# gabrielfnayres/new-vit

Hardware: AMD Instinct MI355X
Metric: volumes_per_sec_mst_dinov2_fwd (higher is better)
Workload: dtype bf16; 1 GPU; MST-DINOv2 (DinoV2ClassifierSlice, ViT-S/14) forward, 4 volumes/GPU of 64x512x512 bf16 zero-padded to 518x518 (N=1370 tokens/slice); global_batch_volumes=4, slices=64, parallelism=single GPU, weights=synthetic (mst.synth seed 2), random init of the reference architecture

## Files before the change

### new-vit_amd/csrc/k_attn16.hip

```cpp
#include <type_traits>

#include "mst_common.h"

namespace {

constexpr float LOG2E = 1.4426950408889634f;
constexpr int KV_TILE_BYTES = 64 * 128;
constexpr int K_ROW = 144, K_TILE_BYTES = 64 * K_ROW;

template <typename T>
__device__ __forceinline__ typename V8<T>::type tr_pair(const char* p_lo, const char* p_hi) {
    typedef typename V8<T>::type vec8;
    union { struct { s16x4 lo, hi; } s; vec8 v; } u;
    u.s.lo = __builtin_amdgcn_ds_read_tr16_b64_v4i16((__attribute__((address_space(3))) s16x4*)(p_lo));
    u.s.hi = __builtin_amdgcn_ds_read_tr16_b64_v4i16((__attribute__((address_space(3))) s16x4*)(p_hi));
    return u.v;
}

constexpr int ATTN_WG_WAVES = 4;
constexpr int WGW = ATTN_WG_WAVES, WGT = 64 * WGW, QB = 32 * WGW;
constexpr int ATTN_WAVES_PER_EU = 4;
template <typename T>
__global__ __launch_bounds__(WGT) __attribute__((amdgpu_waves_per_eu(ATTN_WAVES_PER_EU, ATTN_WAVES_PER_EU))) void attn16_kernel(const T* __restrict__ qkv, T* __restrict__ out,
                                                     int N, int heads, int log2q, int out_blocked) {
    typedef typename V8<T>::type vec8;
    __shared__ __attribute__((aligned(16))) char smem[4 * KV_TILE_BYTES];
    char* const Ks = smem;
    char* const Vs = smem + 2 * KV_TILE_BYTES;

    const int tid = threadIdx.x, lane = tid & 63;
    const int wave = __builtin_amdgcn_readfirstlane(tid >> 6);
    const int nqb = (N + QB - 1) / QB;
    const int tile = xcd_remap(blockIdx.x, gridDim.x);
    const int qb = tile % nqb, h = (tile / nqb) % heads, seq = tile / (nqb * heads);
    const int E = heads * 64, ld = 3 * E;
    const T* base = qkv + (int64_t)seq * N * ld;
    const int h2 = lane >> 5;

    const int q = qb * QB + wave * 32 + (lane & 31);
    const bool wave_active = (qb * QB + wave * 32) < N;
    vec8 bq[4];
    {
        const int qc = q < N ? q : N - 1;
        const T* qp = base + (int64_t)qc * ld + h * 64 + h2 * 8;
#pragma unroll
        for (int ds = 0; ds < 4; ++ds) bq[ds] = *reinterpret_cast<const vec8*>(qp + ds * 16);
    }

    static_assert(WGW == 4 || WGW == 8, "the LDS-DMA staging map deals 16 pieces per tile to 4 or 8 waves");
    constexpr int PPW = 16 / WGW;
    const int d_p0 = wave * PPW;
    const int d_row0 = (d_p0 & 7) * 8 + (lane >> 3);
    const int d_isv = d_p0 >> 3;
    const int d_chunk0 = d_isv ? ((lane & 7) ^ (((d_row0 >> 1) & 1) << 2)) : ((lane & 7) ^ ((d_row0 >> 1) & 7));
    const int d_col0 = (1 + d_isv) * (heads * 64) + h * 64 + d_chunk0 * 8;
    unsigned d_off[PPW];
#pragma unroll
    for (int u = 0; u < PPW; ++u) d_off[u] = (unsigned)(((d_row0 + 8 * u) * ld + ((u & 1) && !d_isv ? (d_col0 ^ 32) : d_col0)) * 2);
    auto dma = [&](int t, int buf) {
        char* dst = (d_isv ? Vs + buf * KV_TILE_BYTES : Ks + buf * KV_TILE_BYTES) + (d_p0 & 7) * 1024;
        if (t * 64 + 64 <= N) {
            const char* tb = reinterpret_cast<const char*>(base) + (int64_t)t * 64 * ld * 2;
#pragma unroll
            for (int u = 0; u < PPW; ++u) {
                const unsigned m0v = (unsigned)(size_t)(__attribute__((address_space(3))) char*)(dst + u * 1024);
#pragma clang diagnostic push
#pragma clang diagnostic ignored "-Winline-asm"
                asm volatile("s_mov_b32 m0, %2\n\ts_nop 0\n\tglobal_load_lds_dwordx4 %0, %1"
                             :
                             : "v"(d_off[u]), "s"(tb), "s"(m0v)
                             : "memory", "m0");
#pragma clang diagnostic pop
            }
        } else {
#pragma unroll
            for (int u = 0; u < PPW; ++u) {
                int key = t * 64 + d_row0 + 8 * u;
                key = key < N ? key : N - 1;
                const int col = (u & 1) && !d_isv ? (d_col0 ^ 32) : d_col0;
                __builtin_amdgcn_global_load_lds(GLB_PTR(base + (int64_t)key * ld + col), LDS_PTR(dst + u * 1024), 16, 0, 0);
            }
        }
    };
    const int krow = lane & 31;
    int k_off4[4];
#pragma unroll
    for (int ds = 0; ds < 4; ++ds) k_off4[ds] = krow * 128 + (((2 * ds + h2) ^ ((krow >> 1) & 7)) << 4);
    const int vi = lane & 15;
    const int vrow = 4 * h2 + (vi >> 2);
    const int vsw = ((vrow >> 1) & 1) << 2;
    const int vchunk = ((lane >> 4) & 1) * 2 + ((vi & 3) >> 1);
    const int v_lane_off = vrow * 128 + (vi & 1) * 8;

    f32x16 oT[2];
#pragma unroll
    for (int r = 0; r < 16; ++r) oT[0][r] = oT[1][r] = 0.f;
    if (!log2q) {
#pragma unroll
        for (int ds = 0; ds < 4; ++ds)
#pragma unroll
            for (int j = 0; j < 8; ++j) bq[ds][j] = (T)((float)bq[ds][j] * LOG2E);
    }
    float r_ref = 0.f, l_run = 0.f;
    constexpr float RT = 8.0f;

    const int nt = (N + 63) >> 6;
    dma(0, 0);
    asm volatile("s_waitcnt vmcnt(0)" ::: "memory");
    __syncthreads();

    constexpr float TH0 = std::is_same<T, f16_t>::value ? 8.0f : 60.0f;
    constexpr float GUARD = std::is_same<T, f16_t>::value ? 32768.0f : 1.2676506e30f;
    bool fast = false;

    auto tile_step = [&](auto mask_tag, auto fast_tag, int t, bool skip_dma) -> bool {
        constexpr bool MASK = decltype(mask_tag)::value;
        constexpr bool FAST = decltype(fast_tag)::value;
        const int buf = t & 1;
        if (t + 1 < nt && !skip_dma) dma(t + 1, buf ^ 1);
        if (wave_active) {
            const char* Kb = Ks + buf * KV_TILE_BYTES;
            const char* Vb = Vs + buf * KV_TILE_BYTES;
            f32x16 s[2];
            const f32x16 zero16 = {0.f, 0.f, 0.f, 0.f, 0.f, 0.f, 0.f, 0.f, 0.f, 0.f, 0.f, 0.f, 0.f, 0.f, 0.f, 0.f};
            const bool upper = !MASK || (t * 64 + 32 < N);
            auto scores = [&](bool with_ref) {
                vec8 kone, qneg;
                if (with_ref) {
#pragma unroll
                    for (int j = 0; j < 8; ++j) kone[j] = qneg[j] = (T)0.f;
                    if (h2 == 0) {
                        kone[0] = (T)1.f;
                        qneg[0] = (T)(-r_ref);
                    }
                }
#pragma unroll
                for (int kb = 0; kb < 2; ++kb) {
                    if (MASK && kb == 1 && !upper) {
#pragma unroll
                        for (int r = 0; r < 16; ++r) s[1][r] = -INFINITY;
                        continue;
                    }
                    s[kb] = with_ref ? mfma32(kone, qneg, zero16) : zero16;
#pragma unroll
                    for (int ds = 0; ds < 4; ++ds) {
                        const vec8 a = *reinterpret_cast<const vec8*>(Kb + k_off4[ds] + kb * 4096);
                        s[kb] = mfma32(a, bq[ds], s[kb]);
                    }
                }
                if constexpr (MASK) {
#pragma unroll
                    for (int kb = 0; kb < 2; ++kb)
#pragma unroll
                        for (int r = 0; r < 16; ++r) {
                            const int key = t * 64 + kb * 32 + (r & 3) + 8 * (r >> 2) + 4 * h2;
                            if (key >= N) s[kb][r] = -INFINITY;
                        }
                }
            };
            float lsum;
            vec8 pf[4];
            auto exps = [&]() {
                lsum = 0.f;
#pragma unroll
                for (int kb = 0; kb < 2; ++kb)
#pragma unroll
                    for (int r = 0; r < 16; ++r) {
                        const float p = __builtin_amdgcn_exp2f(s[kb][r]);
                        s[kb][r] = p;
                        lsum += p;
                    }
#pragma unroll
                for (int ks = 0; ks < 4; ++ks)
#pragma unroll
                    for (int j = 0; j < 8; ++j) pf[ks][j] = (T)s[ks >> 1][(ks & 1) * 8 + j];
            };
            auto classic = [&]() {
                float mx = s[0][0];
#pragma unroll
                for (int r = 1; r < 16; ++r) mx = fmaxf(mx, s[0][r]);
#pragma unroll
                for (int r = 0; r < 16; ++r) mx = fmaxf(mx, s[1][r]);
                {
                    const unsigned mu = __float_as_uint(mx);
                    const auto sw = __builtin_amdgcn_permlane32_swap(mu, mu, false, false);
                    mx = fmaxf(__uint_as_float(sw[0]), __uint_as_float(sw[1]));
                }
                if (t == 0 && __all(fabsf(mx) <= TH0)) {
                    fast = true;
                } else if (t == 0 || !__all(mx <= RT)) {
                    const bool mv = (t == 0) || (mx > RT);
                    const float r_new = mv ? (float)(T)(r_ref + mx) : r_ref;
                    const float delta = r_new - r_ref;
                    const float alpha = t == 0 ? 1.0f : __builtin_amdgcn_exp2f(-delta);
                    r_ref = r_new;
                    l_run *= alpha;
#pragma unroll
                    for (int r = 0; r < 16; ++r) {
                        oT[0][r] *= alpha;
                        oT[1][r] *= alpha;
                        s[0][r] -= delta;
                        s[1][r] -= delta;
                    }
                }
                exps();
            };
            if constexpr (FAST) {
                scores(false);
                exps();
                if (!__all(lsum < GUARD)) return false;
            } else {
                scores(true);
                classic();
            }
            l_run += lsum;
#pragma unroll
            for (int ks = 0; ks < 4; ++ks) {
                if (MASK && ks >= 2 && !upper) continue;
#pragma unroll
                for (int db = 0; db < 2; ++db) {
                    const char* p = Vb + ks * 16 * 128 + v_lane_off + (((db * 4 + vchunk) ^ vsw) * 16);
                    const vec8 vf = tr_pair<T>(p, p + 8 * 128);
                    oT[db] = mfma32(vf, pf[ks], oT[db]);
                }
            }
        }
        asm volatile("s_waitcnt vmcnt(0)" ::: "memory");
        __syncthreads();
        return true;
    };
    const int nt_full = (N & 63) ? nt - 1 : nt;
    const std::false_type FULL{}, CLASSIC{};
    const std::true_type RAGGED{}, FASTM{};
    if (nt_full > 0) tile_step(FULL, CLASSIC, 0, false);
    else tile_step(RAGGED, CLASSIC, 0, false);
    int t = 1;
    bool resume = false;
    if (fast) {
        for (; t < nt_full; ++t)
            if (!tile_step(FULL, FASTM, t, false)) { resume = true; break; }
    }
    for (; t < nt_full; ++t) {
        tile_step(FULL, CLASSIC, t, resume);
        resume = false;
    }
    if (t < nt) tile_step(RAGGED, CLASSIC, t, resume);

    if (wave_active) {
        const float l_tot = l_run + __shfl_xor(l_run, 32, 64);
        const float inv = 1.0f / l_tot;
        if (q < N) {
            const int64_t R = (int64_t)seq * N + q;
            T* op = out_blocked ? out + (R >> 5) * (32 * E) + (4 * h) * 512 + (R & 31) * 8 + 4 * h2
                                : out + R * E + h * 64 + 4 * h2;
            const int sdb = out_blocked ? 1024 : 32, sg2 = out_blocked ? 512 : 16, sg1 = out_blocked ? 256 : 8;
#pragma unroll
            for (int db = 0; db < 2; ++db)
#pragma unroll
                for (int g = 0; g < 4; ++g) {
                    typedef __attribute__((ext_vector_type(4))) T o4;
                    o4 pk;
#pragma unroll
                    for (int e = 0; e < 4; ++e) pk[e] = (T)(oT[db][g * 4 + e] * inv);
                    *reinterpret_cast<o4*>(op + db * sdb + (g >> 1) * sg2 + (g & 1) * sg1) = pk;
                }
        }
    }
}

template <typename T>
__global__ __launch_bounds__(256) void cls_probs_kernel(const T* __restrict__ qkv, float* __restrict__ probs,
                                                        int N, int heads, int hd, int log2q, T* __restrict__ attn_out = nullptr) {
    extern __shared__ float sm[];
    float* q0 = sm;
    float* sc = sm + hd;
    float* red = sc + N;
    const int h = blockIdx.x, seq = blockIdx.y, tid = threadIdx.x;
    const int E = heads * hd, ld = 3 * E;
    const T* base = qkv + (int64_t)seq * N * ld;
    for (int d = tid; d < hd; d += 256) q0[d] = to_f32(base[h * hd + d]);
    __syncthreads();
    float mx = -INFINITY;
    if (hd == 64) {
        const int sub = tid & 7;
        float qr[8];
#pragma unroll
        for (int i = 0; i < 8; ++i) qr[i] = q0[sub * 8 + i];
        for (int j0 = 0; j0 < N; j0 += 32) {
            const int j = j0 + (tid >> 3);
            const T* kp = base + (int64_t)(j < N ? j : N - 1) * ld + E + h * 64 + sub * 8;
            float a = 0.f;
#pragma unroll
            for (int i = 0; i < 8; ++i) a = fmaf(qr[i], to_f32(kp[i]), a);
            a += __shfl_xor(a, 1, 64);
            a += __shfl_xor(a, 2, 64);
            a += __shfl_xor(a, 4, 64);
            if (j < N) {
                if (sub == 0) sc[j] = a;
                mx = fmaxf(mx, a);
            }
        }
    } else {
        for (int j = tid; j < N; j += 256) {
            const T* kp = base + (int64_t)j * ld + E + h * hd;
            float a = 0.f;
            for (int d = 0; d < hd; ++d) a = fmaf(q0[d], to_f32(kp[d]), a);
            sc[j] = a;
            mx = fmaxf(mx, a);
        }
    }
    mx = wave_max(mx);
    if ((tid & 63) == 0) red[tid >> 6] = mx;
    __syncthreads();
    mx = fmaxf(fmaxf(red[0], red[1]), fmaxf(red[2], red[3]));
    float sum = 0.f;
    for (int j = tid; j < N; j += 256) {
        const float p = log2q ? exp2f(sc[j] - mx) : __expf(sc[j] - mx);
        sc[j] = p;
        sum += p;
    }
    sum = wave_sum(sum);
    if ((tid & 63) == 0) red[4 + (tid >> 6)] = sum;
    __syncthreads();
    const float inv = 1.0f / (red[4] + red[5] + red[6] + red[7]);
    if (probs) {
        float* po = probs + ((int64_t)seq * heads + h) * N;
        for (int j = tid; j < N; j += 256) po[j] = sc[j] * inv;
    }
    if (attn_out) {
        float* part = red + 8;
        const int d = tid & 63, pt = tid >> 6;
        const int per = (N + 3) >> 2;
        const int j1 = (pt + 1) * per < N ? (pt + 1) * per : N;
        float a = 0.f;
        for (int j = pt * per; j < j1; ++j) a = fmaf(sc[j], to_f32(base[(int64_t)j * ld + 2 * E + h * 64 + d]), a);
        part[pt * 64 + d] = a;
        __syncthreads();
        if (tid < 64) attn_out[(int64_t)seq * E + h * 64 + tid] = (T)(((part[tid] + part[64 + tid]) + (part[128 + tid] + part[192 + tid])) * inv);
    }
}

template <typename T>
__global__ __launch_bounds__(256) void probs_full_kernel(const T* __restrict__ qkv, float* __restrict__ probs,
                                                         int N, int heads, int hd, int log2q) {
    extern __shared__ float sm[];
    const int lane = threadIdx.x & 63, wave = threadIdx.x >> 6;
    float* qv = sm + wave * (hd + N);
    float* sc = qv + hd;
    const int h = blockIdx.y, seq = blockIdx.z;
    const int qi = blockIdx.x * 4 + wave;
    if (qi >= N) return;
    const int E = heads * hd, ld = 3 * E;
    const T* base = qkv + (int64_t)seq * N * ld;
    for (int d = lane; d < hd; d += 64) qv[d] = to_f32(base[(int64_t)qi * ld + h * hd + d]);
    __builtin_amdgcn_wave_barrier();
    float mx = -INFINITY;
    for (int j = lane; j < N; j += 64) {
        const T* kp = base + (int64_t)j * ld + E + h * hd;
        float a = 0.f;
        for (int d = 0; d < hd; ++d) a = fmaf(qv[d], to_f32(kp[d]), a);
        sc[j] = a;
        mx = fmaxf(mx, a);
    }
    mx = wave_max(mx);
    float sum = 0.f;
    for (int j = lane; j < N; j += 64) {
        const float p = log2q ? exp2f(sc[j] - mx) : __expf(sc[j] - mx);
        sc[j] = p;
        sum += p;
    }
    const float inv = 1.0f / wave_sum(sum);
    float* po = probs + (((int64_t)seq * heads + h) * N + qi) * N;
    for (int j = lane; j < N; j += 64) po[j] = sc[j] * inv;
}

template <typename T>
__global__ __launch_bounds__(256) void probs_full16_kernel(const T* __restrict__ qkv, float* __restrict__ probs, int N,
                                                           int heads, int log2q) {
    typedef typename V8<T>::type vec8;
    __shared__ __attribute__((aligned(16))) char smem[2 * K_TILE_BYTES + 128 * 8];
    char* const Ks = smem;
    float* const stat = reinterpret_cast<float*>(smem + 2 * K_TILE_BYTES);
    const int tid = threadIdx.x, lane = tid & 63;
    const int wave = __builtin_amdgcn_readfirstlane(tid >> 6);
    const int nqb = (N + 127) >> 7;
    const int tile = xcd_remap(blockIdx.x, gridDim.x);
    const int qb = tile % nqb, h = (tile / nqb) % heads, seq = tile / (nqb * heads);
    const int E = heads * 64, ld = 3 * E;
    const T* base = qkv + (int64_t)seq * N * ld;
    const int h2 = lane >> 5;
    const int q = qb * 128 + wave * 32 + (lane & 31);
    const float sc = log2q ? 1.0f : LOG2E;
    vec8 bq[4];
    {
        const int qc = q < N ? q : N - 1;
        const T* qp = base + (int64_t)qc * ld + h * 64 + h2 * 8;
#pragma unroll
        for (int ds = 0; ds < 4; ++ds) bq[ds] = *reinterpret_cast<const vec8*>(qp + ds * 16);
    }
    const int sr = tid >> 2, sc0 = (tid & 3) * 2;
    u32x4 rk0, rk1;
    auto gload = [&](int t) {
        int key = t * 64 + sr;
        key = key < N ? key : N - 1;
        const T* kp = base + (int64_t)key * ld + E + h * 64 + sc0 * 8;
        rk0 = *reinterpret_cast<const u32x4*>(kp);
        rk1 = *reinterpret_cast<const u32x4*>(kp + 8);
    };
    auto lstore = [&](int buf) {
        *reinterpret_cast<u32x4*>(Ks + buf * K_TILE_BYTES + sr * K_ROW + sc0 * 16) = rk0;
        *reinterpret_cast<u32x4*>(Ks + buf * K_TILE_BYTES + sr * K_ROW + sc0 * 16 + 16) = rk1;
    };
    const int k_lane_off = (lane & 31) * K_ROW + h2 * 16;
    const int nt = (N + 63) >> 6;
    const f32x16 zero16 = {0.f, 0.f, 0.f, 0.f, 0.f, 0.f, 0.f, 0.f, 0.f, 0.f, 0.f, 0.f, 0.f, 0.f, 0.f, 0.f};

    float m_run = -INFINITY, l_run = 0.f;
    gload(0);
    lstore(0);
    __syncthreads();
    for (int t = 0; t < nt; ++t) {
        const int buf = t & 1;
        if (t + 1 < nt) gload(t + 1);
        const char* Kb = Ks + buf * K_TILE_BYTES;
        f32x16 s[2];
#pragma unroll
        for (int kb = 0; kb < 2; ++kb) {
            s[kb] = zero16;
#pragma unroll
            for (int ds = 0; ds < 4; ++ds) {
                const vec8 a = *reinterpret_cast<const vec8*>(Kb + k_lane_off + kb * 32 * K_ROW + ds * 32);
                s[kb] = mfma32(a, bq[ds], s[kb]);
            }
        }
        float mx = -INFINITY;
#pragma unroll
        for (int kb = 0; kb < 2; ++kb)
#pragma unroll
            for (int r = 0; r < 16; ++r) {
                const int key = t * 64 + kb * 32 + (r & 3) + 8 * (r >> 2) + 4 * h2;
                s[kb][r] = key < N ? s[kb][r] * sc : -INFINITY;
                mx = fmaxf(mx, s[kb][r]);
            }
        mx = fmaxf(mx, __shfl_xor(mx, 32, 64));
        const float m_new = fmaxf(m_run, mx);
        float lsum = 0.f;
#pragma unroll
        for (int kb = 0; kb < 2; ++kb)
#pragma unroll
            for (int r = 0; r < 16; ++r) lsum += __builtin_amdgcn_exp2f(s[kb][r] - m_new);
        l_run = l_run * __builtin_amdgcn_exp2f(m_run - m_new) + lsum;
        m_run = m_new;
        if (t + 1 < nt) lstore(buf ^ 1);
        __syncthreads();
    }
    {
        const float l_tot = l_run + __shfl_xor(l_run, 32, 64);
        if (h2 == 0) {
            stat[(wave * 32 + (lane & 31)) * 2] = m_run;
            stat[(wave * 32 + (lane & 31)) * 2 + 1] = 1.0f / l_tot;
        }
    }
    __syncthreads();

    float mrow[16], irow[16];
#pragma unroll
    for (int r = 0; r < 16; ++r) {
        const int ql = wave * 32 + (r & 3) + 8 * (r >> 2) + 4 * h2;
        mrow[r] = stat[ql * 2];
        irow[r] = stat[ql * 2 + 1];
    }
    float* const pbase = probs + (((int64_t)seq * heads + h) * N) * N;
    gload(0);
    __syncthreads();
    lstore(0);
    __syncthreads();
    for (int t = 0; t < nt; ++t) {
        const int buf = t & 1;
        if (t + 1 < nt) gload(t + 1);
        const char* Kb = Ks + buf * K_TILE_BYTES;
#pragma unroll
        for (int kb = 0; kb < 2; ++kb) {
            f32x16 s = zero16;
#pragma unroll
            for (int ds = 0; ds < 4; ++ds) {
                const vec8 a = *reinterpret_cast<const vec8*>(Kb + k_lane_off + kb * 32 * K_ROW + ds * 32);
                s = mfma32(bq[ds], a, s);
            }
            const int key = t * 64 + kb * 32 + (lane & 31);
#pragma unroll
            for (int r = 0; r < 16; ++r) {
                const int qq = qb * 128 + wave * 32 + (r & 3) + 8 * (r >> 2) + 4 * h2;
                if (key < N && qq < N) pbase[(int64_t)qq * N + key] = __builtin_amdgcn_exp2f(s[r] * sc - mrow[r]) * irow[r];
            }
        }
        if (t + 1 < nt) lstore(buf ^ 1);
        __syncthreads();
    }
}

}

int launch_attn16(const void* qkv, int dt, int n_seq, int N, int heads, void* out, int log2q, hipStream_t s, int out_blocked) {
    MST_CHECK_ARG(n_seq > 0 && N > 0 && heads > 0, "attention: bad sizes n_seq=%d N=%d heads=%d", n_seq, N, heads);
    const int64_t nwg = (int64_t)((N + QB - 1) / QB) * heads * n_seq;
    MST_CHECK_ARG(nwg < (1ll << 31), "attention: grid too large");
    const dim3 grid((unsigned)nwg), block(WGT);
    if (dt == MST_BF16) attn16_kernel<bf16_t><<<grid, block, 0, s>>>((const bf16_t*)qkv, (bf16_t*)out, N, heads, log2q, out_blocked);
    else if (dt == MST_F16) attn16_kernel<f16_t><<<grid, block, 0, s>>>((const f16_t*)qkv, (f16_t*)out, N, heads, log2q, out_blocked);
    else { mst_set_error("attention16: bad dtype %d", dt); return MST_EINVAL; }
    return mst_check_launch("attention16");
}

int launch_cls_probs(const void* qkv, int dt, int n_seq, int N, int heads, int hd, float* probs, int log2q, hipStream_t s) {
    MST_CHECK_ARG(N > 0 && N <= 12000 && hd > 0 && hd <= 256, "cls_probs: N=%d hd=%d unsupported", N, hd);
    if (n_seq > 65535) {
        const size_t esz = dt == MST_F32 ? 4 : 2;
        for (int s0 = 0; s0 < n_seq; s0 += 65535) {
            const int c = (n_seq - s0 < 65535) ? n_seq - s0 : 65535;
            int rc = launch_cls_probs((const char*)qkv + (size_t)s0 * N * 3 * heads * hd * esz, dt, c, N, heads, hd,
                                      probs + (size_t)s0 * heads * N, log2q, s);
            if (rc) return rc;
        }
        return MST_OK;
    }
    const dim3 grid(heads, n_seq), block(256);
    const size_t sh = (size_t)(hd + N + 8 + 256) * sizeof(float);
    if (dt == MST_BF16) cls_probs_kernel<bf16_t><<<grid, block, sh, s>>>((const bf16_t*)qkv, probs, N, heads, hd, log2q);
    else if (dt == MST_F16) cls_probs_kernel<f16_t><<<grid, block, sh, s>>>((const f16_t*)qkv, probs, N, heads, hd, log2q);
    else if (dt == MST_F32) cls_probs_kernel<float><<<grid, block, sh, s>>>((const float*)qkv, probs, N, heads, hd, log2q);
    else { mst_set_error("cls_probs: bad dtype %d", dt); return MST_EINVAL; }
    return mst_check_launch("cls_probs");
}

int launch_cls_attn(const void* qkv, int dt, int n_seq, int N, int heads, float* probs, void* out, int log2q, hipStream_t s) {
    MST_CHECK_ARG(N > 0 && N <= 12000 && n_seq > 0 && n_seq <= 65535 && out, "cls_attn: N=%d n_seq=%d unsupported", N, n_seq);
    const dim3 grid(heads, n_seq), block(256);
    const size_t sh = (size_t)(64 + N + 8 + 256) * sizeof(float);
    if (dt == MST_BF16) cls_probs_kernel<bf16_t><<<grid, block, sh, s>>>((const bf16_t*)qkv, probs, N, heads, 64, log2q, (bf16_t*)out);
    else if (dt == MST_F16) cls_probs_kernel<f16_t><<<grid, block, sh, s>>>((const f16_t*)qkv, probs, N, heads, 64, log2q, (f16_t*)out);
    else if (dt == MST_F32) cls_probs_kernel<float><<<grid, block, sh, s>>>((const float*)qkv, probs, N, heads, 64, log2q, (float*)out);
    else { mst_set_error("cls_attn: bad dtype %d", dt); return MST_EINVAL; }
    return mst_check_launch("cls_attn");
}

int launch_probs_full(const void* qkv, int dt, int n_seq, int N, int heads, int hd, float* probs, int log2q, hipStream_t s) {
    if (hd == 64 && (dt == MST_BF16 || dt == MST_F16)) {
        MST_CHECK_ARG(N > 0 && n_seq > 0 && heads > 0, "probs_full: bad sizes");
        const int64_t nwg = (int64_t)((N + 127) / 128) * heads * n_seq;
        MST_CHECK_ARG(nwg < (1ll << 31), "probs_full: grid too large");
        if (dt == MST_BF16) probs_full16_kernel<bf16_t><<<dim3((unsigned)nwg), dim3(256), 0, s>>>((const bf16_t*)qkv, probs, N, heads, log2q);
        else probs_full16_kernel<f16_t><<<dim3((unsigned)nwg), dim3(256), 0, s>>>((const f16_t*)qkv, probs, N, heads, log2q);
        return mst_check_launch("probs_full16");
    }
    MST_CHECK_ARG(N > 0 && N <= 3800 && hd > 0 && hd <= 256, "probs_full: N=%d hd=%d unsupported", N, hd);
    if (n_seq > 65535) {
        const size_t esz = dt == MST_F32 ? 4 : 2;
        for (int s0 = 0; s0 < n_seq; s0 += 65535) {
            const int c = (n_seq - s0 < 65535) ? n_seq - s0 : 65535;
            int rc = launch_probs_full((const char*)qkv + (size_t)s0 * N * 3 * heads * hd * esz, dt, c, N, heads, hd,
                                       probs + (size_t)s0 * heads * N * N, log2q, s);
            if (rc) return rc;
        }
        return MST_OK;
    }
    const dim3 grid((N + 3) / 4, heads, n_seq), block(256);
    const size_t sh = (size_t)4 * (hd + N) * sizeof(float);
    if (dt == MST_BF16) probs_full_kernel<bf16_t><<<grid, block, sh, s>>>((const bf16_t*)qkv, probs, N, heads, hd, log2q);
    else if (dt == MST_F16) probs_full_kernel<f16_t><<<grid, block, sh, s>>>((const f16_t*)qkv, probs, N, heads, hd, log2q);
    else if (dt == MST_F32) probs_full_kernel<float><<<grid, block, sh, s>>>((const float*)qkv, probs, N, heads, hd, log2q);
    else { mst_set_error("probs_full: bad dtype %d", dt); return MST_EINVAL; }
    return mst_check_launch("probs_full");
}
```

Measured before the change: 163.5 volumes/s.

## Unroll attention KV loop by two with static buffers and MFMA row-sum

Unrolls the attention tile loop in pairs so the double-buffer index is a compile-time constant, hoists the V fragment offsets, and prefetches the first V fragments before the overflow guard check in the fast path. The softmax row sum moves from a scalar add chain plus a cross-lane shuffle to small MFMAs against a lane-selection vector. Inactive waves now run a separate loop that only issues DMA and barriers. The aim is to cut address arithmetic, VALU reduction work and the latency exposed at the guard. The cost is more control-flow complexity and a risk of barrier mismatch between active and inactive waves.

```diff
diff --git a/new-vit_amd/csrc/k_attn16.hip b/new-vit_amd/csrc/k_attn16.hip
--- a/new-vit_amd/csrc/k_attn16.hip
+++ b/new-vit_amd/csrc/k_attn16.hip
@@ -91,6 +91,10 @@
     const int vsw = ((vrow >> 1) & 1) << 2;
     const int vchunk = ((lane >> 4) & 1) * 2 + ((vi & 3) >> 1);
     const int v_lane_off = vrow * 128 + (vi & 1) * 8;
+    const int v_off2[2] = {v_lane_off + ((vchunk ^ vsw) << 4), v_lane_off + (((4 + vchunk) ^ vsw) << 4)};
+    vec8 sel;
+#pragma unroll
+    for (int j = 0; j < 8; ++j) sel[j] = (((lane >> 2) & 1) == ((lane >> 4) & 1)) ? (T)1.f : (T)0.f;
 
     f32x16 oT[2];
 #pragma unroll
@@ -113,12 +117,12 @@
     constexpr float GUARD = std::is_same<T, f16_t>::value ? 32768.0f : 1.2676506e30f;
     bool fast = false;
 
-    auto tile_step = [&](auto mask_tag, auto fast_tag, int t, bool skip_dma) -> bool {
+    auto tile_step = [&](auto mask_tag, auto fast_tag, auto buf_tag, int t, bool skip_dma) -> bool {
         constexpr bool MASK = decltype(mask_tag)::value;
         constexpr bool FAST = decltype(fast_tag)::value;
-        const int buf = t & 1;
+        const int buf = decltype(buf_tag)::value < 0 ? (t & 1) : decltype(buf_tag)::value;
         if (t + 1 < nt && !skip_dma) dma(t + 1, buf ^ 1);
-        if (wave_active) {
+        {
             const char* Kb = Ks + buf * KV_TILE_BYTES;
             const char* Vb = Vs + buf * KV_TILE_BYTES;
             f32x16 s[2];
@@ -158,22 +162,23 @@
                         }
                 }
             };
-            float lsum;
             vec8 pf[4];
+            f32x4 lsum;
             auto exps = [&]() {
-                lsum = 0.f;
 #pragma unroll
                 for (int kb = 0; kb < 2; ++kb)
 #pragma unroll
-                    for (int r = 0; r < 16; ++r) {
-                        const float p = __builtin_amdgcn_exp2f(s[kb][r]);
-                        s[kb][r] = p;
-                        lsum += p;
-                    }
+                    for (int r = 0; r < 16; ++r) s[kb][r] = __builtin_amdgcn_exp2f(s[kb][r]);
 #pragma unroll
                 for (int ks = 0; ks < 4; ++ks)
 #pragma unroll
                     for (int j = 0; j < 8; ++j) pf[ks][j] = (T)s[ks >> 1][(ks & 1) * 8 + j];
+                lsum = f32x4{0.f, 0.f, 0.f, 0.f};
+#pragma unroll
+                for (int ks = 0; ks < 4; ++ks) {
+                    if (MASK && ks >= 2 && !upper) continue;
+                    lsum = mfma16(sel, pf[ks], lsum);
+                }
             };
             auto classic = [&]() {
                 float mx = s[0][0];
@@ -205,22 +210,30 @@
                 }
                 exps();
             };
+            auto vfrag = [&](int ks, int db) {
+                const char* p = Vb + ks * 16 * 128 + v_off2[db];
+                return tr_pair<T>(p, p + 8 * 128);
+            };
             if constexpr (FAST) {
                 scores(false);
                 exps();
-                if (!__all(lsum < GUARD)) return false;
             } else {
                 scores(true);
                 classic();
             }
-            l_run += lsum;
+            vec8 vf0[2];
+            if constexpr (FAST) {
+                vf0[0] = vfrag(0, 0);
+                vf0[1] = vfrag(0, 1);
+                if (!__all(lsum[0] < GUARD)) return false;
+            }
+            l_run += lsum[0];
 #pragma unroll
             for (int ks = 0; ks < 4; ++ks) {
                 if (MASK && ks >= 2 && !upper) continue;
 #pragma unroll
                 for (int db = 0; db < 2; ++db) {
-                    const char* p = Vb + ks * 16 * 128 + v_lane_off + (((db * 4 + vchunk) ^ vsw) * 16);
-                    const vec8 vf = tr_pair<T>(p, p + 8 * 128);
+                    const vec8 vf = FAST && ks == 0 ? vf0[db] : vfrag(ks, db);
                     oT[db] = mfma32(vf, pf[ks], oT[db]);
                 }
             }
@@ -230,25 +243,53 @@
         return true;
     };
     const int nt_full = (N & 63) ? nt - 1 : nt;
+    if (!wave_active) {
+        for (int t = 0; t < nt; ++t) {
+            if (t + 1 < nt) dma(t + 1, (t + 1) & 1);
+            asm volatile("s_waitcnt vmcnt(0)" ::: "memory");
+            __syncthreads();
+        }
+        return;
+    }
     const std::false_type FULL{}, CLASSIC{};
     const std::true_type RAGGED{}, FASTM{};
-    if (nt_full > 0) tile_step(FULL, CLASSIC, 0, false);
-    else tile_step(RAGGED, CLASSIC, 0, false);
+    const std::integral_constant<int, 0> B0{};
+    const std::integral_constant<int, 1> B1{};
+    const std::integral_constant<int, -1> BDYN{};
+    if (nt_full > 0) tile_step(FULL, CLASSIC, B0, 0, false);
+    else tile_step(RAGGED, CLASSIC, B0, 0, false);
     int t = 1;
     bool resume = false;
     if (fast) {
-        for (; t < nt_full; ++t)
-            if (!tile_step(FULL, FASTM, t, false)) { resume = true; break; }
-    }
-    for (; t < nt_full; ++t) {
-        tile_step(FULL, CLASSIC, t, resume);
+        for (; t + 1 < nt_full; t += 2) {
+            int ok1 = __builtin_amdgcn_readfirstlane((int)tile_step(FULL, FASTM, B1, t, false)), ok2 = 0;
+            asm volatile("" : "+s"(ok1));
+            if (ok1) ok2 = (int)tile_step(FULL, FASTM, B0, t + 1, false);
+            ok2 = __builtin_amdgcn_readfirstlane(ok2);
+            asm volatile("" : "+s"(ok2));
+            if (!ok2) { t += ok1; resume = true; break; }
+        }
+        if (!resume && t < nt_full) {
+            if (tile_step(FULL, FASTM, B1, t, false)) ++t;
+            else resume = true;
+        }
+    }
+    if (t < nt_full && !(t & 1)) {
+        tile_step(FULL, CLASSIC, B0, t, resume);
         resume = false;
-    }
-    if (t < nt) tile_step(RAGGED, CLASSIC, t, resume);
-
-    if (wave_active) {
-        const float l_tot = l_run + __shfl_xor(l_run, 32, 64);
-        const float inv = 1.0f / l_tot;
+        ++t;
+    }
+    while (t < nt_full) {
+        tile_step(FULL, CLASSIC, B1, t, resume);
+        resume = false;
+        if (++t == nt_full) break;
+        tile_step(FULL, CLASSIC, B0, t, false);
+        ++t;
+    }
+    if (t < nt) tile_step(RAGGED, CLASSIC, BDYN, t, resume);
+
+    {
+        const float inv = 1.0f / l_run;
         if (q < N) {
             const int64_t R = (int64_t)seq * N + q;
             T* op = out_blocked ? out + (R >> 5) * (32 * E) + (4 * h) * 512 + (R & 31) * 8 + 4 * h2
```

Result: no change. 164.9 volumes/s, median of 6 (+0.9%).
